# sourcedennis/wasm-pathtracer

Hardware: AMD Instinct MI355X
Metric: Mray/s (primary+shadow+bounce) at 1920x1080, 1/2/4/8 GPU; L2 vs CPU ref (higher is better)
Workload: dtype f32; 1 GPU; C3 bunny scene (scene id 2), 1920x1080, 64 spp per GPU share (64 spp frame), depth 8, NormalNEE; rays=25682600955, parallelism=single GPU

## Files before the change

include/wpt.h:

```cpp
#ifndef WPT_H
#define WPT_H

#include <stddef.h>
#include <stdint.h>

#ifdef __cplusplus
extern "C" {
#endif

#define WPT_OK 0
#define WPT_ERR_NOT_INIT (-1)
#define WPT_ERR_ALREADY_INIT (-2)
#define WPT_ERR_INVALID_SCENE (-3)
#define WPT_ERR_INVALID_ARG (-4)
#define WPT_ERR_UNSUPPORTED (-5)
#define WPT_ERR_DEVICE (-6)
#define WPT_ERR_NO_MESH (-7)

#define WPT_NO_NEE 0
#define WPT_NORMAL_NEE 1
#define WPT_PNEE 2


int wpt_init(uint32_t width, uint32_t height, uint32_t scene_id, float cam_x, float cam_y, float cam_z,
// ... 85 lines not shown
#define WPT_OPT_TRAVERSAL_SH 2
#define WPT_OPT_FUSED 3
#define WPT_OPT_FUSED_BELOW 4
#define WPT_OPT_SMALL_LANES 5
#define WPT_OPT_PIXEL_TILE 6
#define WPT_OPT_GRID_PCT 7
#define WPT_OPT_REFILL 8
#define WPT_OPT_REFILL_SH 9
#define WPT_OPT_TREELET 10
#define WPT_OPT_BVH_BUILD 11
#define WPT_OPT_LANES 12
#define WPT_OPT_FINISH_BELOW 13
#define WPT_OPT_TRACE_GRID_PCT 14
#define WPT_OPT_FINISH_EVERY 20
#define WPT_OPT_PROBE 22
#define WPT_OPT_STOCK 23
#define WPT_OPT_STOCK_LANES 24
#define WPT_OPT_FILL 25
#define WPT_OPT_ASYNC_PRIO 26
#define WPT_OPT_ASYNC_GRID_PCT 27
#define WPT_OPT_STOCK_AHEAD 30
#define WPT_OPT_STOCK_EVERY 32
#define WPT_OPT_STOCK_EXTRA 33
#define WPT_OPT_ASYNC_ONESHOT 31
#define WPT_OPT_STOCK_PREFILL 35
#define WPT_OPT_ASYNC_FUSED_BELOW 36
#define WPT_OPT_PRESOLVE 37
#define WPT_OPT_DROP_MISS 38
#define WPT_OPT_PRESOLVE_SHADOW 39
#define WPT_OPT_GEN_SHADE 40
#define WPT_OPT_STOCK_RANKS 42
#define WPT_OPT_STOCK_RING_BYTES 43
#define WPT_OPT_VIEWPORT 44
#define WPT_OPT_LOG 34
#define WPT_OPT_SCENE_TRAVERSAL 28
#define WPT_OPT_OCT_VIEW 41
#define WPT_OPT_SCENE_TRI_ONLY 29
int wpt_set_option(int32_t option, int64_t value);
int64_t wpt_probe_read(uint32_t* meta, uint32_t* rec, uint64_t* rec_entries, double* ticks_per_us);
int wpt_get_option(int32_t option, int64_t* value);
int wpt_scene_build_info(double* out);
int wpt_clear_stats(void);
int wpt_sync(void);
int wpt_bvh_depth(void);

int wpt_trace_rays(size_t n, const float* rays, float* t_out, int32_t* id_out);
int wpt_shadow_rays(size_t n, const float* pq, const int32_t* light, uint8_t* occluded);
int wpt_first_hit(uint32_t sample, float* dir3, float* t, int32_t* id, uint32_t* visits,
                  float* normal3, float* albedo3, uint8_t* kind);
int wpt_primary_rays(uint32_t width, uint32_t height, const float* cam5, uint32_t frame_seed,
                     uint32_t sample, float* rays6);
int wpt_presolve_rays(size_t n, const float* rays, uint8_t* resolved, float* t_out, int32_t* id_out);
int wpt_presolve_shadow_rays(size_t n, const float* pq, const int32_t* light, uint8_t* resolved);

int wpt_shutdown(void);

void* wpt_debug_scene_new(int32_t scene_id, const float* mesh_vertices, size_t num_vertices);
int wpt_debug_scene_info(void* h, uint64_t* out);
int wpt_debug_scene_nodes4(void* h, uint32_t* out);
int wpt_debug_scene_nodes(void* h, uint32_t* out);
int wpt_debug_scene_shapes(void* h, float* out);
int wpt_debug_scene_materials(void* h, float* out);
int wpt_debug_scene_lights(void* h, uint32_t* out);
int wpt_debug_scene_presolve(void* h, size_t n, const float* rays, uint8_t* resolved, float* t_out, int32_t* id_out);
int wpt_debug_scene_guards(void* h, uint32_t* num_guards, float* boxes, uint32_t* leaf_guard);
int wpt_debug_scene_presolve_shadow(void* h, size_t n, const float* pq, const int32_t* light, uint8_t* resolved);
// ... 11 lines not shown
```

wasm-pathtracer_amd/csrc/wpt_render.h:

```cpp
#pragma once
#include <hip/hip_runtime.h>
#include <stdint.h>
#include <string>
#include <algorithm>
#include <deque>
#include <vector>

#include "wpt_photon.h"
#include "wpt_scene.h"
#include "wpt_seqsum.h"

namespace wpt {

constexpr int kMaxInf = 16;
constexpr int kMaxBvhDepth = 4096;
constexpr int kMaxBounces = 512;

struct DevScene {
  const float4* nodes;
  const float4* tree;
  uint32_t tree_pairs, tree_root_lf;
  const float4* prims;
  const uint32_t* kinds;
  const float4* all;
  const uint32_t* all_kinds;
  const float4* mats;
  const float4* lights;
  const float4* nodes4;
  const uint32_t* leaf_table;
  uint32_t num_inf, num_finite, num_shapes, num_lights;
  uint32_t use_bvh, tri_only;
  uint32_t refill_lanes;
  uint32_t refill_lanes_sh;
  int stack_cap;
  uint32_t* overflow;
  const uint32_t* oct_child;
  const float* oct_cum;
  const uint32_t* oct_corners;
  uint32_t oct_nodes;
  uint32_t oct_lds_words;
  float bg[3];
  float4 planes[kMaxInf];
  uint4* probe;
  const PresolveBoxes* pre;
};

struct Stats {
  uint64_t paths = 0;
  uint64_t rays = 0;
  uint64_t shadow_rays = 0;
  uint64_t node_visits = 0;
  uint64_t prim_tests = 0;
  uint64_t bounces = 0;
  uint64_t ext_visits = 0, ext_tests = 0, ext_node_bytes = 0;
  uint64_t sh_visits = 0, sh_tests = 0, sh_node_bytes = 0;
  uint64_t fallback_ext = 0, fallback_sh = 0;
  uint64_t ex_body_lanes = 0, ex_bodies = 0, lf_body_lanes = 0, lf_bodies = 0;
  uint64_t ext_lane_iters = 0, ext_live_iters = 0, sh_lane_iters = 0, sh_live_iters = 0;
  uint64_t photon_rays = 0, photons = 0;
  uint64_t trace_bytes = 0;
  uint64_t max_ray_visits = 0;
  uint64_t sum_chunks = 0, sum_resummed = 0, sum_fetched = 0;
  uint64_t finish_paths = 0, finish_max_bounces = 0;
  uint64_t stock_traced = 0, stock_consumed = 0, fill_paths = 0;
  uint64_t stock_deficit = 0, stock_waits = 0, plan_us = 0, stock_us = 0;
  uint64_t stock_rays = 0;
  uint64_t stock_rays_used = 0;
// ... 349 lines not shown
  uint64_t xslot_ = 0;
  uint64_t maxpart_ = 0;
  uint32_t* d_xidx_ = nullptr;
  bool photons_ok_ = false;
  uint64_t photons_shot_ = 0, photons_stored_ = 0;
  std::vector<uint32_t> oct_child_;
  std::vector<float> oct_cum_;
  uint32_t* d_oct_child_ = nullptr;
  float* d_oct_cum_ = nullptr;
  uint32_t* d_oct_corners_ = nullptr;

  int device_ = -1;
  int ncu_ = 256;
  static constexpr int kTravVariants = 8;
  uint32_t grid_ext_[2 * kTravVariants] = {};
  uint32_t grid_sh_[2 * kTravVariants] = {};
  uint32_t grid_tr_[4] = {};
  uint32_t grid_shade_ = 512;
  uint32_t shade_occ_[32] = {};
  size_t shade_occ_smem_[32] = {};
  bool fused_ = false;
  uint64_t fused_below_ = 1ull << 24;
  int small_lanes_ = 2;
  int traversal_ = 3, traversal_sh_ = 3;
  int trav_ext_ = 0, trav_sh_ = 0;
  bool treelet_ = true;
  uint32_t pixel_tile_ = 8;
  int grid_pct_ = 50;
#ifndef WPT_TRACE_GRID_PCT
#define WPT_TRACE_GRID_PCT 75
#endif
  int trace_grid_pct_ = WPT_TRACE_GRID_PCT;
  uint32_t refill_ = 12, refill_sh_ = 16;
  uint64_t finish_below_ = 1u << 18;
  int finish_every_ = 4;
  uint32_t num_guards_ = 0;
  uint32_t light_guards_ = 0;
  bool presolve_ = true;
  bool drop_miss_ = true;
  bool presolve_shadow_ = true;
  bool gen_shade_ = true;
  uint32_t gen_shade_occ_[2] = {};
  uint32_t probe_cap_ = 0, probe_waves_ = 0, probe_used_ = 0;
  uint4* d_probe_ = nullptr;
  std::vector<uint32_t> probe_meta_;
  uint4* probe_slot(const LaunchCtx& C, int kernel, uint32_t grid);
  uint32_t* d_fallback_ = nullptr;
  void* d_fh_ = nullptr;
  size_t fh_cap_ = 0;
  uint2* d_fh_spill_ = nullptr;
  size_t fh_spill_cap_ = 0;
  hipStream_t stream_ = nullptr;
  PathSet lanes_[kMaxLanes];
  int lanes_made_ = 0;
  bool stats_pending_ = false;
  int pend_nl_ = 0, pend_b_ = 0;
  bool pend_stock_ = false, pend_presolve_ = false;
  int nlanes_ = 4;
  hipEvent_t ev_main_ = nullptr;
  hipEvent_t ev_ref_ = nullptr;
  std::vector<void*> scene_bufs_;
  DevScene ds_{};
  uint32_t depth_ = 0;
  bool scene_ok_ = false;

  uint32_t w_ = 0, h_ = 0;
// ... 38 lines not shown
```

wasm-pathtracer_amd/csrc/wpt_render.hip:

```cpp
#include "wpt_render.h"
#include "wpt_partition.h"
#include "wpt_photon.h"
#include "wpt_quartic.h"
#include "wpt_seqsum.h"

#include <algorithm>
#include <chrono>
#include <cstdlib>
#include <cmath>
#include <cstdio>
#include <cstring>
#include <deque>
#include <memory>
#include <mutex>
#include <unordered_map>
#include <thread>
#include <type_traits>

#define HIP_OK(expr)                                                     \
  do {                                                                   \
    hipError_t e_ = (expr);                                              \
    if (e_ != hipSuccess) {                                              \
      err = std::string(#expr " failed: ") + hipGetErrorString(e_);      \
      return false;                                                      \
// ... 301 lines not shown
  h.root_b = S.nodes[1];
  if (kTreePairs > 0) {
    for (uint32_t i = threadIdx.x; i < 4 * S.tree_pairs; i += kTBlock) {
      const float4 v = S.tree[i];
      tree[i] = f4v{v.x, v.y, v.z, v.w};
    }
    if (S.tree_pairs != 0) h.root_b.z = __uint_as_float(S.tree_root_lf);
  }
  h.gtree = gtree;
  const bool fits = S.num_lights <= kLdsLights;
  if (fits && threadIdx.x < 4 * S.num_lights) {
    const uint32_t l = threadIdx.x >> 2, w = threadIdx.x & 3u;
    const uint32_t sid = __float_as_uint(S.lights[5 * l + 1].w);
    const float4 v = S.prims[4 * (size_t)(sid - S.num_inf) + w];
    lrec[4 * threadIdx.x] = v.x;
    lrec[4 * threadIdx.x + 1] = v.y;
    lrec[4 * threadIdx.x + 2] = v.z;
    lrec[4 * threadIdx.x + 3] = v.w;
    if (w == 0) lid[l] = (int32_t)sid;
  }
  __syncthreads();
  h.lrec = fits ? lrec : nullptr;
  h.lid = lid;
  return h;
}

template <bool COUNT>
__device__ __forceinline__ bool enter_root(const DevScene& S, const Hot& H, Lane& L, uint32_t& visits,
                                           uint32_t& nbytes) {
  if (COUNT) { visits++; nbytes += 32; }
  const float4 a = H.root_a, b = H.root_b;
  float h;
  if (!box_entry(a, b, L.o, L.inv, L.best, h)) return false;
  L.lf = __float_as_uint(b.z);
  L.cnt = __float_as_uint(b.w);
  L.sp = 0;
  return true;
}

typedef __attribute__((address_space(3))) uint32_t lds_u32;
typedef __attribute__((address_space(3))) float lds_f32;
struct Stack {
  lds_u32* code;
  lds_f32* h;
  uint2* spill;
  uint32_t stride;
  int cap;
  uint32_t* overflow;
};

__device__ __forceinline__ uint32_t encode_child(uint32_t lf, uint32_t cnt, uint32_t node) {
  const uint32_t leaf = (cnt < 128u && lf < (1u << 24)) ? (0x80000000u | (cnt << 24) | lf) : (0x40000000u | node);
  return cnt == 0 ? lf : leaf;
}

__device__ __forceinline__ void stack_store(const Stack& st, int k, uint32_t code, float h) {
  if (k < kLdsSlots) {
    st.code[k * kTBlock] = code;
    st.h[k * kTBlock] = h;
  } else {
    st.spill[(size_t)(k - kLdsSlots) * st.stride] = make_uint2(code, __float_as_uint(h));
  }
}

__device__ __forceinline__ void stack_load(const Stack& st, int k, uint32_t& code, float& h) {
  if (k < kLdsSlots) {
    code = st.code[k * kTBlock];
    h = st.h[k * kTBlock];
// ... 1058 lines not shown
    cnt[0] = (uint32_t)__popcll(fm);
    const OutMasks M = count_out<true>(R, V, cnt + 1);
    cnt[4] = ShadeFields::pack((uint32_t)__popcll(__ballot(drop0)), (uint32_t)__popcll(__ballot(shaded)));
    if (lane == 0) A.publish(wid, cnt);
    __syncthreads();
    if (wid == 0)
      A.reserve(lane,
                {{3, false, ~0u}, {0, false, ~0u}, {0, true, ~0u}, {1, false, ShadeFields::kMask}, {-1, false, 0u}},
                [&](const uint32_t(&incl)[5]) {
                  const uint32_t tf = A.total(incl[0]), te = A.total(incl[4]);
                  auto t = shade_take<BA>(lane, reinterpret_cast<u64*>(counts + 2), incl[1], incl[2], A.total(incl[3]));
                  if (lane == kWaves + 2)
                    t = A.take(counts, tf, 0u, true);
                  else if (lane == kWaves + 3)
                    t = A.take(counts + kResWord, 0u, ShadeFields::get(te, 0), true);
                  else if (lane == kWaves + 4)
                    t = A.take(counts + kGenShadeWord, ShadeFields::top(te, 1), 0u, true);
                  t.go = t.go && t.inc != 0ull;
                  return t;
                });
    __syncthreads();
    if (front0) {
      const uint32_t p = A.at(0, wid, (uint32_t)__popcll(fm & below));
      s0.thr[p] = R.th;
      s0.o[p] = R.ro;
      s0.d[p] = R.rd;
    } else
      store_out<true, 1>(A, wid, below, M, R, V, out, sh, col, t_nx, id_nx, n);
    __syncthreads();
  }
}

struct WaveFeed {
  uint32_t n, v, wave, nwaves;
  __device__ WaveFeed(uint32_t n_) : n(n_), v(0) {
    wave = (blockIdx.x * kTBlock + threadIdx.x) >> 6;
    nwaves = (gridDim.x * kTBlock) >> 6;
  }
  static constexpr uint32_t K = kFeedChunk;
  __device__ uint32_t pos(uint32_t k) const { return ((k / K) * nwaves + wave) * K + (k % K); }
  __device__ bool more() const { return pos(v) < n; }
  __device__ uint32_t taken() const { return taken_below(n); }
  __device__ uint32_t taken_below(uint32_t m) const {
    const uint32_t C = m / K, rem = m % K;
    const uint32_t full = C > wave ? (C - wave - 1u) / nwaves + 1u : 0u;
    const uint32_t part = (rem != 0u && C % nwaves == wave) ? rem : 0u;
    return min(v, full * K + part);
  }
  __device__ uint32_t take(uint64_t take_m) {
    const uint32_t rank = (uint32_t)__popcll(take_m & ((1ull << (threadIdx.x & 63)) - 1ull));
    const uint32_t p = pos(v + rank);
    v += (uint32_t)__popcll(take_m);
    return p;
  }
};

template <int OCT>
__global__ void __launch_bounds__(kShadeBlock) k_photon_sample(DevScene S, uint32_t n, const float* __restrict__ pts,
                                                               const uint32_t* __restrict__ st_in,
                                                               uint32_t* __restrict__ light, float* __restrict__ pdf,
                                                               uint32_t* __restrict__ st_out) {
  extern __shared__ uint32_t s_oct[];
  const OctView<OCT> O = oct_view<OCT>(S, s_oct);
  __syncthreads();
  for (uint32_t i = blockIdx.x * kShadeBlock + threadIdx.x; i < n; i += gridDim.x * kShadeBlock) {
    uint32_t s = st_in[i], li = 0;
    float p = 0.0f;
    photon_sample(S, O, s, mk(pts[3 * (size_t)i], pts[3 * (size_t)i + 1], pts[3 * (size_t)i + 2]), li, p);
    light[i] = li;
    pdf[i] = p;
    st_out[i] = s;
  }
}

__global__ void __launch_bounds__(kBlock) k_photon_gen(DevScene S, uint32_t seed, uint32_t k0, uint32_t n,
                                                       float4* __restrict__ ro, float4* __restrict__ rd,
                                                       float4* __restrict__ rec) {
  const uint32_t i = blockIdx.x * kBlock + threadIdx.x;
  if (i >= n) return;
  uint32_t s = photon_seed(seed, k0 + i);
  const uint32_t li = xs_next_in_range(s, S.num_lights);
  const float4* L = S.lights + 5 * (size_t)li;
  const float4 L0 = L[0], L1 = L[1], L2 = L[2], L3 = L[3], L4 = L[4];
  const float q1 = xs_next(s);
  const float q2 = xs_next(s);
  const float q1s = sqrtf(q1);
// ... 65 lines not shown
    const uint32_t f = (uint32_t)__popcll(__ballot(live && L.cnt != 0));
    ex_lanes += e;
    ex_bodies += e ? 1u : 0u;
    lf_lanes += f;
    lf_bodies += f ? 1u : 0u;
  }
  __device__ __forceinline__ void flush(unsigned long long* work, int ca, int cb) const {
    work_add_wave(work, ca, 64ull * it);
    work_add_wave(work, ca + 1, live_a);
    if (cb >= 0) {
      work_add_wave(work, cb, 64ull * it);
      work_add_wave(work, cb + 1, live_b);
    }
    work_add_wave(work, 10, ex_lanes);
    work_add_wave(work, 11, ex_bodies);
    work_add_wave(work, 12, lf_lanes);
    work_add_wave(work, 13, lf_bodies);
  }
};

template <bool TRI_ONLY, bool COUNT, int TRAV>
__global__ void WPT_TRACE_BOUNDS k_extend(DevScene S, const float4* __restrict__ ro,
                                                   const float4* __restrict__ rd, const uint32_t* __restrict__ count,
                                                   float* __restrict__ t_out, int32_t* __restrict__ id_out,
                                                   uint2* __restrict__ spill, unsigned long long* work,
                                                   uint32_t* fallbacks) {
  constexpr bool FAST = TRAV == 1;
  __shared__ uint32_t s_code[kLdsSlots * kTBlock];
  __shared__ float s_h[kLdsSlots * kTBlock];
  __shared__ float s_lrec[16 * kLdsLights];
  __shared__ int32_t s_lid[kLdsLights];
  __shared__ f4v s_tree[4 * kTreePairs + 1];
  const uint32_t n = *count;
  const Hot H = load_hot(S, (lds_f32h*)s_lrec, (lds_i32*)s_lid, (lds_f4v*)s_tree, (const float4*)s_tree);
  const uint32_t G = gridDim.x * kTBlock;
  const Stack stk{(lds_u32*)(s_code + threadIdx.x), (lds_f32*)(s_h + threadIdx.x),
                  spill + blockIdx.x * kTBlock + threadIdx.x, G, S.stack_cap, S.overflow};
  uint32_t visits = 0, tests = 0, nbytes = 0;
  WaveFeed feed(n);
  const uint32_t p_t0 = S.probe ? probe_now() : 0u;
  uint32_t p_dry = 0u;
  Lane L;
  uint32_t slot = 0;
  bool live = false;
  bool fast = FAST;
  bool tie = false, quirk = false, dummy = false;
  BodyLanes bodies;
  const float inf = __int_as_float(0x7f800000);
  for (;;) {
    const uint64_t idle_m = __ballot(!live);
    const uint32_t nidle = (uint32_t)__popcll(idle_m);
    if (nidle != 0 && (nidle >= S.refill_lanes || nidle == 64u) && feed.more()) {
      const uint32_t q0 = feed.take(idle_m);
      const bool got = q0 < n;
      if (S.probe && p_dry == 0u && !feed.more()) p_dry = probe_now();
      if (!live && got) {
        slot = q0;
        fast = FAST;
        tie = quirk = false;
        const float4 o4 = ro[slot], d4 = rd[slot];
        live = begin_extend<TRI_ONLY, COUNT, FAST>(S, H, L, ld3(o4), ld3(d4), visits, tests, nbytes);
        if (!live) st_hit(t_out + slot, id_out + slot, L.best_id >= 0 ? L.best : inf, L.best_id);
      }
    }
    if (!__any(live) && !feed.more()) {
      if (S.probe) probe_close(S, p_t0, p_dry, feed.taken());
      break;
    }
    if (COUNT) bodies.count(live, false, L);
    if (live) {
      const bool more = (FAST && fast)
                            ? step4<false, TRI_ONLY, COUNT>(S, L, stk, -1, 0.0f, dummy, tie, quirk, visits, tests, nbytes)
                            : step<false, TRI_ONLY, COUNT>(S, H, L, stk, -1, 0.0f, dummy, visits, tests, nbytes);
      if (!more) {
        live = false;
        if (FAST && fast && (tie || quirk)) {
          fast = false;
          atomicAdd(fallbacks, 1u);
          live = begin_extend<TRI_ONLY, COUNT, false>(S, H, L, L.o, L.d, visits, tests, nbytes);
        }
        if (!live) st_hit(t_out + slot, id_out + slot, L.best_id >= 0 ? L.best : inf, L.best_id);
      }
    }
  }
  if (COUNT) {
    work_add(work, 0, visits);
    work_add(work, 1, tests);
    work_add(work, 2, nbytes);
    bodies.flush(work, 6, -1);
  }
}

__device__ __forceinline__ void add_contribution(float4* __restrict__ col, float4 c) {
  const uint32_t path = __float_as_uint(c.w);
  float4 v = col[path];
  v.x += c.x;
  v.y += c.y;
  v.z += c.z;
  col[path] = v;
}

template <bool TRI_ONLY, bool COUNT, int TRAV>
__global__ void WPT_TRACE_BOUNDS k_shadow(DevScene S, const uint32_t* __restrict__ count,
                                                   const float4* __restrict__ so, const float4* __restrict__ sd,
                                                   const float4* __restrict__ sc, float4* __restrict__ col,
                                                   uint8_t* __restrict__ occ_out, uint2* __restrict__ spill,
                                                   unsigned long long* work, uint32_t* fallbacks) {
  constexpr bool FAST = TRAV == 1;
  __shared__ uint32_t s_code[kLdsSlots * kTBlock];
  __shared__ float s_h[kLdsSlots * kTBlock];
  __shared__ float s_lrec[16 * kLdsLights];
  __shared__ int32_t s_lid[kLdsLights];
  __shared__ f4v s_tree[4 * kTreePairs + 1];
  const uint32_t n = *count;
  const Hot H = load_hot(S, (lds_f32h*)s_lrec, (lds_i32*)s_lid, (lds_f4v*)s_tree, (const float4*)s_tree);
  const uint32_t G = gridDim.x * kTBlock;
  const Stack stk{(lds_u32*)(s_code + threadIdx.x), (lds_f32*)(s_h + threadIdx.x),
                  spill + blockIdx.x * kTBlock + threadIdx.x, G, S.stack_cap, S.overflow};
  uint32_t visits = 0, tests = 0, nbytes = 0;
  WaveFeed feed(n);
  const uint32_t p_t0 = S.probe ? probe_now() : 0u;
  uint32_t p_dry = 0u;
  Lane L;
  uint32_t cur = 0;
  float dir_len = 0.0f, early = 0.0f;
  int32_t light = -1;
  bool occluded = false;
  bool live = false;
  bool fast = FAST;
  bool tie = false, quirk = false;
  BodyLanes bodies;
  for (;;) {
    bool finished = false;
    const uint64_t idle_m = __ballot(!live);
    const uint32_t nidle = (uint32_t)__popcll(idle_m);
    if (nidle != 0 && (nidle >= S.refill_lanes_sh || nidle == 64u) && feed.more()) {
      const uint32_t q0 = feed.take(idle_m);
      const bool got = q0 < n;
      if (S.probe && p_dry == 0u && !feed.more()) p_dry = probe_now();
      if (!live && got) {
        cur = q0;
        const float4 o4 = so[cur], d4 = sd[cur];
        dir_len = o4.w;
        light = (int32_t)__float_as_uint(d4.w);
        fast = FAST;
        tie = quirk = false;
        live = begin_shadow<TRI_ONLY, COUNT, FAST>(S, H, L, ld3(o4), ld3(d4), dir_len, light, early, occluded, visits,
                                                   tests, nbytes);
        finished = !live;
      }
    }
    if (!__any(live || finished) && !feed.more()) {
      if (S.probe) probe_close(S, p_t0, p_dry, feed.taken());
      break;
    }
    if (COUNT) bodies.count(live, false, L);
    if (live) {
      const bool more =
          (FAST && fast)
              ? step4<true, TRI_ONLY, COUNT>(S, L, stk, light, early, occluded, tie, quirk, visits, tests, nbytes)
              : step<true, TRI_ONLY, COUNT>(S, H, L, stk, light, early, occluded, visits, tests, nbytes);
      if (!more) {
        live = false;
        finished = true;
        if (FAST && fast && !occluded && (tie || quirk)) {
          fast = false;
          atomicAdd(fallbacks + 1, 1u);
          if (begin_shadow<TRI_ONLY, COUNT, false>(S, H, L, L.o, L.d, dir_len, light, early, occluded, visits, tests,
                                                   nbytes)) {
            live = true;
            finished = false;
          }
// ... 2 lines not shown
    }
    if (finished) {
      const bool occ = shadow_verdict(L, dir_len, light, occluded);
      if (occ_out) occ_out[cur] = occ ? 1 : 0;
      else if (!occ) add_contribution(col, sc[cur]);
    }
  }
  if (COUNT) {
    work_add(work, 3, visits);
    work_add(work, 4, tests);
    work_add(work, 5, nbytes);
    bodies.flush(work, 8, -1);
  }
}

template <bool TRI_ONLY, bool COUNT>
#ifndef WPT_FUSED_WAVES
#define WPT_FUSED_WAVES 8
#endif
__global__ void __launch_bounds__(kTBlock, TRI_ONLY ? WPT_FUSED_WAVES : 1) k_trace(DevScene S, const float4* __restrict__ ro,
                                                  const float4* __restrict__ rd, const uint32_t* __restrict__ cnt_ext,
                                                  float* __restrict__ t_out, int32_t* __restrict__ id_out,
                                                  const uint32_t* __restrict__ cnt_sh, const float4* __restrict__ so,
                                                  const float4* __restrict__ sd, const float4* __restrict__ sc,
                                                  float4* __restrict__ col, uint2* __restrict__ spill,
                                                  unsigned long long* work) {
  __shared__ uint32_t s_code[kLdsSlots * kTBlock];
  __shared__ float s_h[kLdsSlots * kTBlock];
  __shared__ float s_lrec[16 * kLdsLights];
  __shared__ int32_t s_lid[kLdsLights];
  __shared__ f4v s_tree[4 * kTreePairs + 1];
  const uint32_t ne = *cnt_ext;
  const uint32_t n = ne + *cnt_sh;
  const Hot H = load_hot(S, (lds_f32h*)s_lrec, (lds_i32*)s_lid, (lds_f4v*)s_tree, (const float4*)s_tree);
  const uint32_t G = gridDim.x * kTBlock;
  const Stack stk{(lds_u32*)(s_code + threadIdx.x), (lds_f32*)(s_h + threadIdx.x),
                  spill + blockIdx.x * kTBlock + threadIdx.x, G, S.stack_cap, S.overflow};
  uint32_t ev = 0, et = 0, eb = 0, sv = 0, st = 0, sb = 0, cv = 0, ct = 0, cb = 0, vmax = 0;
  WaveFeed feed(n);
  const uint32_t p_t0 = S.probe ? probe_now() : 0u;
  uint32_t p_dry = 0u;
  Lane L;
  uint32_t slot = 0;
  bool live = false, is_sh = false, occluded = false;
  BodyLanes bodies;
  float dir_len = 0.0f, early = -__int_as_float(0x7f800000);
  int32_t light = -1;
  const float inf = __int_as_float(0x7f800000);
  for (;;) {
    bool finished = false;
    const uint64_t idle_m = __ballot(!live);
    const uint32_t nidle = (uint32_t)__popcll(idle_m);
    if (nidle != 0 && (nidle >= S.refill_lanes || nidle == 64u) && feed.more()) {
      const uint32_t q0 = feed.take(idle_m);
      const bool got = q0 < n;
      if (!live && got) {
        is_sh = q0 >= ne;
        slot = is_sh ? q0 - ne : q0;
      }
      if (S.probe && p_dry == 0u && !feed.more()) p_dry = probe_now();
      if (!live && got) {
        const float4 o4 = is_sh ? so[slot] : ro[slot];
        const float4 d4 = is_sh ? sd[slot] : rd[slot];
        if (!is_sh) {
          light = -1;
          early = -inf;
          occluded = false;
          live = begin_extend<TRI_ONLY, COUNT, false>(S, H, L, ld3(o4), ld3(d4), cv, ct, cb);
        } else {
          dir_len = o4.w;
          light = (int32_t)__float_as_uint(d4.w);
          live = begin_shadow<TRI_ONLY, COUNT, false>(S, H, L, ld3(o4), ld3(d4), dir_len, light, early, occluded, cv,
                                                      ct, cb);
        }
        finished = !live;
      }
    }
    if (!__any(live || finished) && !feed.more()) {
      if (S.probe) probe_close(S, p_t0, p_dry, feed.taken());
      break;
    }
    if (COUNT) bodies.count(live, is_sh, L);
    if (live) {
      if (!step<true, TRI_ONLY, COUNT>(S, H, L, stk, light, early, occluded, cv, ct, cb)) {
        live = false;
        finished = true;
      }
    }
    if (finished) {
      if (!is_sh) st_hit(t_out + slot, id_out + slot, L.best_id >= 0 ? L.best : inf, L.best_id);
      else if (!shadow_verdict(L, dir_len, light, occluded)) add_contribution(col, sc[slot]);
      if (COUNT) {
        vmax = max(vmax, cv);
// ... 470 lines not shown
  if (!up(all.data(), all.size() * sizeof(float4), &p)) return false;
  ds.all = (const float4*)p;
  if (!up(all_kinds.data(), all_kinds.size() * sizeof(uint32_t), &p)) return false;
  ds.all_kinds = (const uint32_t*)p;
  if (!up(mats.data(), mats.size() * sizeof(float4), &p)) return false;
  ds.mats = (const float4*)p;
  if (!up(lights.data(), lights.size() * sizeof(float4), &p)) return false;
  ds.lights = (const float4*)p;
  {
    const size_t n4 = std::max<size_t>(sc.nodes4.size(), 1);
    std::vector<Node4> n4v(n4);
    if (!sc.nodes4.empty()) memcpy(n4v.data(), sc.nodes4.data(), sizeof(Node4) * sc.nodes4.size());
    if (!up(n4v.data(), sizeof(Node4) * n4, &p)) return false;
    ds.nodes4 = (const float4*)p;
    std::vector<uint32_t> lt(std::max<size_t>(sc.leaf_table.size(), 2), 0u);
    std::copy(sc.leaf_table.begin(), sc.leaf_table.end(), lt.begin());
    if (!up(lt.data(), sizeof(uint32_t) * lt.size(), &p)) return false;
    ds.leaf_table = (const uint32_t*)p;
    auto mode = [&](int want) {
      const bool b4 = want == 1 || (want == 3 && !sc.tri_only && sc.use_bvh);
      return (b4 && !sc.nodes4.empty()) ? 1 : 0;
    };
    trav_ext_ = mode(traversal_);
    trav_sh_ = mode(traversal_sh_);
  }
  ds.num_inf = sc.num_inf;
  ds.num_finite = (uint32_t)nf;
  ds.num_shapes = (uint32_t)ns;
  ds.num_lights = (uint32_t)sc.lights.size();
  ds.use_bvh = sc.use_bvh ? 1u : 0u;
  ds.tri_only = sc.tri_only ? 1u : 0u;
  ds.refill_lanes = refill_;
  ds.refill_lanes_sh = refill_sh_;
  for (int k = 0; k < 3; k++) ds.bg[k] = sc.background[k];
  for (uint32_t i = 0; i < sc.num_inf && i < (uint32_t)kMaxInf; i++) ds.planes[i] = all[4 * i];
  {
    PresolveBoxes pre{};
    if (sc.use_bvh && nf != 0) pre = sc.pre;
    if (!up(&pre, sizeof pre, &p)) return false;
    ds.pre = (const PresolveBoxes*)p;
    num_guards_ = pre.num_guards;
    light_guards_ = pre.light_guards;
  }
  ds_ = ds;
  depth_ = sc.depth;
  ds_.stack_cap = (int)std::max<uint32_t>(sc.depth + 2, 3 * sc.depth4 + 4);
  ds_.overflow = d_fallback_ + 2;
  if (!size_grids(err)) return false;
  scene_ok_ = true;
  return true;
}

bool Renderer::set_option(int opt, int64_t v, std::string& err) {
  auto range = [&](int64_t lo, int64_t hi) {
    if (v < lo || v > hi) {
      err = "option value out of range";
      return false;
    }
    return true;
  };
  switch (opt) {
    case 1:
    case 2:
      if (!range(0, 3) || v == 2) { err = "traversal: 0 (bvh2), 1 (bvh4) or 3 (auto)"; return false; }
      (opt == 1 ? traversal_ : traversal_sh_) = (int)v;
      return true;
// ... 11 lines not shown
    case 12:
      if (!set_lanes((int)v)) { err = "lanes out of range"; return false; }
      return true;
    case 13: if (!range(0, (int64_t)1 << 32)) return false; finish_below_ = (uint64_t)v; return true;
    case 14:
      if (!range(1, 100)) return false;
      trace_grid_pct_ = (int)v;
      return !stream_ || size_grids(err);
    case 20: if (!range(1, 64)) return false; finish_every_ = (int)v; return true;
    case 23:
      if (v != 0 && (v < 64 || v > 4096 || (v & (v - 1)) != 0)) { err = "stock: 0 or a power of two 64..4096"; return false; }
      if (!drain_async(err)) return false;
      stock_drop();
      stock_slots_ = (uint32_t)v;
      return true;
    case 42:
      if (!range(0, 1)) return false;
      if (!drain_async(err)) return false;
      stock_drop();
      stock_ranks_ = v != 0;
      return true;
    case 25: if (!range(0, 1)) return false; fill_on_ = v != 0; return true;
    case 30: if (!range(0, 64)) return false; stock_ahead_ = (uint32_t)v; return true;
    case 32: if (!range(1, 1024)) return false; stock_every_ = (uint32_t)v; return true;
    case 33: if (!range(0, 64)) return false; stock_extra_ = (uint32_t)v; return true;
    case 31: if (!range(0, 1)) return false; async_oneshot_ = v != 0; return true;
    case 34: if (!range(0, 1)) return false; log_ = (int)v; return true;
    case 35: if (!range(0, 1)) return false; stock_prefill_ = v != 0; return true;
    case 36: if (!range(0, (int64_t)1 << 40)) return false; async_fused_below_ = (uint64_t)v; return true;
    case 37: if (!range(0, 1)) return false; presolve_ = v != 0; return true;
    case 38: if (!range(0, 1)) return false; drop_miss_ = v != 0; return true;
    case 39: if (!range(0, 1)) return false; presolve_shadow_ = v != 0; return true;
    case 40: if (!range(0, 1)) return false; gen_shade_ = v != 0; return true;
    case 26:
      if (!range(0, 1)) return false;
      if (!drain_async(err)) return false;
      async_prio_ = (int)v;
      return true;
    case 27: if (!range(0, 100)) return false; async_grid_pct_ = (int)v; return true;
    case 28:
    case 29:
    case 41:
    case 43:
    case 44: err = "read-only option"; return false;
    case 24:
      if (!range(1, kMaxLanes - kAsyncLane0 - 1)) return false;
      if (!drain_async(err)) return false;
      stock_lanes_ = (int)v;
      refill_lane_ = 0;
      return true;
    case 22:
      if (!range(0, 1 << 20)) return false;
      probe_cap_ = (uint32_t)v;
      probe_used_ = 0;
      probe_meta_.clear();
      if (d_probe_) { (void)hipFree(d_probe_); d_probe_ = nullptr; }
      return true;
    default: err = "unknown option"; return false;
  }
}

bool Renderer::get_option(int opt, int64_t& v) const {
  switch (opt) {
    case 1: v = traversal_; return true;
    case 2: v = traversal_sh_; return true;
    case 3: v = fused_ ? 1 : 0; return true;
    case 4: v = (int64_t)fused_below_; return true;
    case 5: v = small_lanes_; return true;
    case 6: v = pixel_tile_; return true;
    case 7: v = grid_pct_; return true;
    case 8: v = refill_; return true;
    case 9: v = refill_sh_; return true;
    case 10: v = treelet_ ? 1 : 0; return true;
    case 12: v = nlanes_; return true;
    case 13: v = (int64_t)finish_below_; return true;
    case 14: v = trace_grid_pct_; return true;
    case 20: v = finish_every_; return true;
    case 22: v = probe_cap_; return true;
    case 23: v = stock_slots_; return true;
    case 25: v = fill_on_ ? 1 : 0; return true;
    case 30: v = stock_ahead_; return true;
    case 32: v = stock_every_; return true;
    case 33: v = stock_extra_; return true;
    case 31: v = async_oneshot_ ? 1 : 0; return true;
    case 34: v = log_; return true;
    case 35: v = stock_prefill_ ? 1 : 0; return true;
    case 36: v = (int64_t)async_fused_below_; return true;
    case 37: v = presolve_ ? 1 : 0; return true;
    case 38: v = drop_miss_ ? 1 : 0; return true;
    case 39: v = presolve_shadow_ ? 1 : 0; return true;
    case 40: v = gen_shade_ ? 1 : 0; return true;
    case 26: v = async_prio_; return true;
    case 27: v = async_grid_pct_; return true;
    case 28: v = !scene_ok_ ? -1 : !ds_.use_bvh ? 2 : trav_ext_; return true;
    case 29: v = !scene_ok_ ? -1 : ds_.tri_only ? 1 : 0; return true;
    case 41: v = !photons_ok_ ? -1 : ds_.oct_lds_words == 0 ? 0 : (ds_.oct_lds_words > ds_.oct_nodes ? 2 : 1); return true;
    case 24: v = stock_lanes_; return true;
    case 42: v = stock_ranks_ ? 1 : 0; return true;
    case 43: v = (int64_t)ring_bytes(); return true;
    case 44: v = (int64_t)w_ | ((int64_t)h_ << 32); return true;
    default: return false;
  }
}

bool Renderer::set_viewport(uint32_t w, uint32_t h, std::string& err) {
  if (!stream_) { err = "no device"; return false; }
  if (w == 0 || h == 0) { err = "empty viewport"; return false; }
  if (!drain_async(err)) return false;
  stock_drop();
  HIP_OK(hipStreamSynchronize(stream_));
  w_ = w;
  h_ = h;
  free_rounds();
  if (d_acc_) (void)hipFree(d_acc_);
  if (d_cnt_) (void)hipFree(d_cnt_);
  if (d_rgba_) (void)hipFree(d_rgba_);
  if (d_samp_) (void)hipFree(d_samp_);
  d_acc_ = nullptr; d_cnt_ = nullptr; d_rgba_ = nullptr; d_samp_ = nullptr;
  HIP_OK(hipMalloc(&d_acc_, sizeof(float4) * (size_t)w * h));
  HIP_OK(hipMalloc(&d_cnt_, sizeof(uint32_t) * (size_t)w * h));
  HIP_OK(hipMalloc(&d_rgba_, 4 * (size_t)w * h));
  HIP_OK(hipMalloc(&d_samp_, 4 * (size_t)w * h));
  return set_partition(rank_, nranks_, tile_, err);
}
// ... 1188 lines not shown
}

bool Renderer::read_radiance(float* acc3, uint32_t* cnt, std::string& err) {
  const size_t np = (size_t)w_ * h_;
  std::vector<float4> a(np);
  HIP_OK(hipMemcpyAsync(a.data(), d_acc_, sizeof(float4) * np, hipMemcpyDeviceToHost, stream_));
  if (cnt) HIP_OK(hipMemcpyAsync(cnt, d_cnt_, sizeof(uint32_t) * np, hipMemcpyDeviceToHost, stream_));
  HIP_OK(hipStreamSynchronize(stream_));
  for (size_t i = 0; i < np; i++) {
    acc3[3 * i] = a[i].x;
    acc3[3 * i + 1] = a[i].y;
    acc3[3 * i + 2] = a[i].z;
  }
  return true;
}

bool Renderer::copy_partition(float* dev_dst, std::string& err) {
  const uint32_t n = (uint32_t)part_pix_.size();
  k_pack_partition<<<blocks_for(n), kBlock, 0, stream_>>>(nranks_ > 1 ? d_part_pix_ : nullptr, n, d_acc_, d_cnt_,
                                                          (float4*)dev_dst);
  HIP_OK(hipGetLastError());
  HIP_OK(hipStreamSynchronize(stream_));
  return true;
}

bool Renderer::launch_extend(const LaunchCtx& C, const float4* ro, const float4* rd, const uint32_t* cnt,
                             std::string& err) {
  const PathSet& L = *C.ps;
  const int v = (ds_.tri_only ? 1 : 0) | (C.count ? 2 : 0) | (trav_ext_ << 2);
  const int full = C.batch_lanes == 1 ? kTravVariants : 0;
  const uint32_t g = std::min(async_grid(C, grid_ext_[v + full], 100), spill_grid(L));
  DevScene ds = ds_;
  ds.probe = probe_slot(C, 1, g);
#define WPT_EXT(T, CN, F)                                                                                     \
  k_extend<T, CN, F><<<g, kTBlock, 0, C.stream>>>(ds, ro, rd, cnt, L.hit_t(C.hit_sel), L.hit_id(C.hit_sel), \
                                                 L.spill, d_work_, d_fallback_)
  switch (v) {
    case 0: LAUNCH_TIMED(C, 1, extend, n_extend, WPT_EXT(false, false, 0)); break;
    case 1: LAUNCH_TIMED(C, 1, extend, n_extend, WPT_EXT(true, false, 0)); break;
    case 2: LAUNCH_TIMED(C, 1, extend, n_extend, WPT_EXT(false, true, 0)); break;
    case 3: LAUNCH_TIMED(C, 1, extend, n_extend, WPT_EXT(true, true, 0)); break;
    case 4: LAUNCH_TIMED(C, 1, extend, n_extend, WPT_EXT(false, false, 1)); break;
    case 5: LAUNCH_TIMED(C, 1, extend, n_extend, WPT_EXT(true, false, 1)); break;
    case 6: LAUNCH_TIMED(C, 1, extend, n_extend, WPT_EXT(false, true, 1)); break;
    default: LAUNCH_TIMED(C, 1, extend, n_extend, WPT_EXT(true, true, 1)); break;
  }
#undef WPT_EXT
  if (ds.probe && C.probe_res) {
    k_probe_add<<<1, 1, 0, C.stream>>>(ds.probe, C.probe_res);
    if (C.bounce == 0) k_probe_add_sh<<<1, 1, 0, C.stream>>>(ds.probe, L.counts + kGenShadeWord);
    HIP_OK(hipGetLastError());
  }
  return true;
}

bool Renderer::launch_shadow(const LaunchCtx& C, const uint32_t* cnt, uint8_t* occ_out, std::string& err) {
  const PathSet& L = *C.ps;
  const int v = (ds_.tri_only ? 1 : 0) | (C.count ? 2 : 0) | (trav_sh_ << 2);
  const int full = C.batch_lanes == 1 ? kTravVariants : 0;
  const uint32_t g = std::min(async_grid(C, grid_sh_[v + full], 100), spill_grid(L));
  DevScene ds = ds_;
  ds.probe = probe_slot(C, 3, g);
#define WPT_SH(T, CN, F)                                                                                        \
  k_shadow<T, CN, F><<<g, kTBlock, 0, C.stream>>>(ds, cnt, L.so, L.sd, L.sc, L.col, occ_out, L.spill, d_work_, \
                                                 d_fallback_)
  switch (v) {
    case 0: LAUNCH_TIMED(C, 3, shadow, n_shadow, WPT_SH(false, false, 0)); break;
    case 1: LAUNCH_TIMED(C, 3, shadow, n_shadow, WPT_SH(true, false, 0)); break;
    case 2: LAUNCH_TIMED(C, 3, shadow, n_shadow, WPT_SH(false, true, 0)); break;
    case 3: LAUNCH_TIMED(C, 3, shadow, n_shadow, WPT_SH(true, true, 0)); break;
    case 4: LAUNCH_TIMED(C, 3, shadow, n_shadow, WPT_SH(false, false, 1)); break;
    case 5: LAUNCH_TIMED(C, 3, shadow, n_shadow, WPT_SH(true, false, 1)); break;
    case 6: LAUNCH_TIMED(C, 3, shadow, n_shadow, WPT_SH(false, true, 1)); break;
    default: LAUNCH_TIMED(C, 3, shadow, n_shadow, WPT_SH(true, true, 1)); break;
  }
#undef WPT_SH
  if (ds.probe && C.probe_res) {
    k_probe_add_sh<<<1, 1, 0, C.stream>>>(ds.probe, cnt + (kShResWord - 3));
    HIP_OK(hipGetLastError());
  }
  return true;
}

bool Renderer::launch_trace(const LaunchCtx& C, std::string& err) {
  const PathSet& L = *C.ps;
  const int b = C.bounce;
  const int v = (ds_.tri_only ? 1 : 0) | (C.count ? 2 : 0);
  const uint32_t g = std::min(async_grid(C, grid_tr_[v], trace_grid_pct_, 2), spill_grid(L));
  DevScene ds = ds_;
  ds.probe = probe_slot(C, 5, g);
#define WPT_TR(T, CN)                                                                                          \
  k_trace<T, CN><<<g, kTBlock, 0, C.stream>>>(ds, L.ro[b & 1], L.rd[b & 1], L.ext_count(b), L.hit_t(C.hit_sel), \
                                             L.hit_id(C.hit_sel), L.sh_count(b - 1), L.so, L.sd, L.sc, L.col,  \
                                             L.spill, d_work_)
  switch (v) {
    case 0: LAUNCH_TIMED(C, 5, trace, n_trace, WPT_TR(false, false)); break;
    case 1: LAUNCH_TIMED(C, 5, trace, n_trace, WPT_TR(true, false)); break;
    case 2: LAUNCH_TIMED(C, 5, trace, n_trace, WPT_TR(false, true)); break;
    default: LAUNCH_TIMED(C, 5, trace, n_trace, WPT_TR(true, true)); break;
  }
#undef WPT_TR
  if (ds.probe && C.probe_res) {
    k_probe_add<<<1, 1, 0, C.stream>>>(ds.probe, C.probe_res);
    k_probe_add_sh<<<1, 1, 0, C.stream>>>(ds.probe, L.sh_count(b - 1) + (kShResWord - 3));
    HIP_OK(hipGetLastError());
  }
  return true;
}

uint4* Renderer::probe_slot(const LaunchCtx& C, int kernel, uint32_t grid) {
  if (probe_used_ >= probe_cap_) return nullptr;
  const uint32_t waves = grid * (kTBlock / 64);
  if (!d_probe_) {
    probe_waves_ = max_grid() * (kTBlock / 64);
    const uint64_t cap_max = (1ull << 28) / std::max<uint32_t>(probe_waves_, 1);
    probe_cap_ = (uint32_t)std::min<uint64_t>(probe_cap_, cap_max);
    if (hipMalloc(&d_probe_, sizeof(uint4) * (size_t)probe_waves_ * probe_cap_) != hipSuccess) {
      d_probe_ = nullptr;
      probe_cap_ = 0;
      return nullptr;
    }
  }
  if (waves > probe_waves_) return nullptr;
// ... 827 lines not shown
```

wasm-pathtracer_amd/interface.py:

```python
import ctypes

import numpy as np

from ._lib import lib

OK = 0
ERR_NOT_INIT, ERR_ALREADY_INIT, ERR_INVALID_SCENE, ERR_INVALID_ARG = -1, -2, -3, -4
ERR_UNSUPPORTED, ERR_DEVICE, ERR_NO_MESH = -5, -6, -7
NO_NEE, NORMAL_NEE, PNEE = 0, 1, 2


class WptError(RuntimeError):
    def __init__(self, code, msg):
        super().__init__(f"[{code}] {msg}")
        self.code = code


def _check(rc):
    if rc < 0:
        raise WptError(rc, lib().wpt_last_error().decode())
    return rc


def init(width, height, scene_id, cam_x, cam_y, cam_z, cam_rot_x, cam_rot_y):
# ... 241 lines not shown
    out = (ctypes.c_double * 28)()
    _check(lib().wpt_kernel_times(ctypes.addressof(out), 28))
    names = ("generate", "extend", "shade", "shadow", "accumulate", "trace")
    kt = {n: {"ms": out[2 * i], "launches": int(out[2 * i + 1]), "busy_ms": out[12 + 2 * i],
              "logical_launches": int(out[13 + 2 * i])} for i, n in enumerate(names)}
    return kt


def set_counting(on):
    _check(lib().wpt_set_counting(1 if on else 0))


def set_profiling(on):
    _check(lib().wpt_set_profiling(1 if on else 0))


def scene_build_info():
    out = (ctypes.c_double * 2)()
    _check(lib().wpt_scene_build_info(ctypes.addressof(out)))
    return float(out[0]), bool(out[1])


def set_lanes(n):
    _check(lib().wpt_set_lanes(int(n)))


OPTIONS = {"defaults": 0, "traversal": 1, "traversal_sh": 2, "fused": 3, "fused_below": 4, "small_lanes": 5, "pixel_tile": 6,
           "grid_pct": 7, "refill": 8, "refill_sh": 9, "treelet": 10, "bvh_build": 11, "lanes": 12,
           "finish_below": 13, "trace_grid_pct": 14, "finish_every": 20, "probe": 22, "stock": 23, "stock_lanes": 24,
           "fill": 25, "async_prio": 26, "async_grid_pct": 27, "scene_traversal": 28, "scene_tri_only": 29,
           "stock_ahead": 30, "async_oneshot": 31, "stock_every": 32, "stock_extra": 33,
           "log": 34, "stock_prefill": 35, "async_fused_below": 36, "presolve": 37, "drop_miss": 38,
           "presolve_shadow": 39, "gen_shade": 40, "oct_view": 41,
           "stock_ranks": 42, "stock_ring_bytes": 43, "viewport": 44}
TRAVERSALS = {"bvh2": 0, "bvh4": 1, "auto": 3}
OPTION_VALUES = {"traversal": TRAVERSALS, "traversal_sh": TRAVERSALS,
                 "bvh_build": {"auto": 0, "host": 1, "gpu": 2}}


def set_option(name, value):
    if isinstance(value, str) and not value.lstrip("-").isdigit():
        value = OPTION_VALUES[name][value]
    _check(lib().wpt_set_option(OPTIONS[name], int(value)))


def get_option(name):
    v = ctypes.c_int64(0)
    _check(lib().wpt_get_option(OPTIONS[name], ctypes.addressof(v)))
    return v.value


def probe_read():
    L = lib()
    ent = ctypes.c_uint64(0)
    tpu = ctypes.c_double(0.0)
    n = L.wpt_probe_read(None, None, ctypes.addressof(ent), ctypes.addressof(tpu))
    if n < 0:
        raise WptError(int(n), L.wpt_last_error().decode())
    meta = np.zeros((n, 5), np.uint32)
    rec = np.zeros((ent.value, 4), np.uint32)
    if n:
        ent.value = rec.shape[0]
        _check(L.wpt_probe_read(meta.ctypes.data, rec.ctypes.data, ctypes.addressof(ent), ctypes.addressof(tpu)))
    return meta, rec, tpu.value


def clear_stats():
# ... 157 lines not shown
```

Before: 10090 Mray/s.

## Size wave feed to work count and retire surplus blocks early

```diff
diff --git a/include/wpt.h b/include/wpt.h
--- a/include/wpt.h
+++ b/include/wpt.h
@@ -141,6 +141,7 @@
 #define WPT_OPT_STOCK_RANKS 42
 #define WPT_OPT_STOCK_RING_BYTES 43
 #define WPT_OPT_VIEWPORT 44
+#define WPT_OPT_FEED_MIN_CHUNKS 45
 #define WPT_OPT_LOG 34
 #define WPT_OPT_SCENE_TRAVERSAL 28
 #define WPT_OPT_OCT_VIEW 41
diff --git a/wasm-pathtracer_amd/csrc/wpt_feed.h b/wasm-pathtracer_amd/csrc/wpt_feed.h
--- /dev/null
+++ b/wasm-pathtracer_amd/csrc/wpt_feed.h
@@ -0,0 +1,39 @@
+#pragma once
+#include <stdint.h>
+
+#if defined(__HIPCC__)
+#include <hip/hip_runtime.h>
+#define WPT_FEED_HD __host__ __device__ __forceinline__
+#else
+#define WPT_FEED_HD inline
+#endif
+
+namespace wpt {
+
+constexpr uint32_t kFeedMinChunksMax = 4096;
+
+WPT_FEED_HD uint32_t feed_waves(uint32_t n, uint32_t nwaves, uint32_t block_waves, uint32_t c, uint32_t K) {
+  const uint32_t per = K * c;
+  const uint32_t want = n / per + (n % per != 0u ? 1u : 0u);
+  const uint32_t blocks = want > block_waves ? (want + block_waves - 1u) / block_waves : 1u;
+  const uint32_t wa = blocks * block_waves;
+  return wa < nwaves ? wa : nwaves;
+}
+
+WPT_FEED_HD uint32_t feed_pos(uint32_t wa, uint32_t w, uint32_t k, uint32_t K) {
+  return ((k / K) * wa + w) * K + (k % K);
+}
+
+WPT_FEED_HD uint32_t feed_taken_below(uint32_t wa, uint32_t w, uint32_t v, uint32_t m, uint32_t K) {
+  const uint32_t C = m / K, rem = m % K;
+  const uint32_t full = C > w ? (C - w - 1u) / wa + 1u : 0u;
+  const uint32_t part = (rem != 0u && C % wa == w) ? rem : 0u;
+  const uint32_t own = full * K + part;
+  return v < own ? v : own;
+}
+
+WPT_FEED_HD uint32_t feed_own(uint32_t wa, uint32_t w, uint32_t n, uint32_t K) {
+  return feed_taken_below(wa, w, 0xFFFFFFFFu, n, K);
+}
+
+}
diff --git a/wasm-pathtracer_amd/csrc/wpt_render.h b/wasm-pathtracer_amd/csrc/wpt_render.h
--- a/wasm-pathtracer_amd/csrc/wpt_render.h
+++ b/wasm-pathtracer_amd/csrc/wpt_render.h
@@ -6,6 +6,7 @@
 #include <deque>
 #include <vector>
 
+#include "wpt_feed.h"
 #include "wpt_photon.h"
 #include "wpt_scene.h"
 #include "wpt_seqsum.h"
@@ -33,6 +34,7 @@
   uint32_t refill_lanes;
   uint32_t refill_lanes_sh;
   int stack_cap;
+  uint32_t feed_min_chunks;
   uint32_t* overflow;
   const uint32_t* oct_child;
   const float* oct_cum;
@@ -448,6 +450,8 @@
 #endif
   int trace_grid_pct_ = WPT_TRACE_GRID_PCT;
   uint32_t refill_ = 12, refill_sh_ = 16;
+  uint32_t feed_min_chunks_ = 1;
+  uint32_t feed_chunks(const LaunchCtx& C) const { return C.async && async_oneshot_ ? 1u : feed_min_chunks_; }
   uint64_t finish_below_ = 1u << 18;
   int finish_every_ = 4;
   uint32_t num_guards_ = 0;
diff --git a/wasm-pathtracer_amd/csrc/wpt_render.hip b/wasm-pathtracer_amd/csrc/wpt_render.hip
--- a/wasm-pathtracer_amd/csrc/wpt_render.hip
+++ b/wasm-pathtracer_amd/csrc/wpt_render.hip
@@ -357,8 +357,14 @@
   const float4 a = H.root_a, b = H.root_b;
   float h;
   if (!box_entry(a, b, L.o, L.inv, L.best, h)) return false;
-  L.lf = __float_as_uint(b.z);
-  L.cnt = __float_as_uint(b.w);
+  if (S.tree_pairs != 0) {
+    L.lf = S.tree_root_lf;
+    L.cnt = 0;
+  } else {
+    const float4 rb = S.nodes[1];
+    L.lf = __float_as_uint(rb.z);
+    L.cnt = __float_as_uint(rb.w);
+  }
   L.sp = 0;
   return true;
 }
@@ -1483,26 +1489,25 @@
 }
 
 struct WaveFeed {
-  uint32_t n, v, wave, nwaves;
-  __device__ WaveFeed(uint32_t n_) : n(n_), v(0) {
-    wave = (blockIdx.x * kTBlock + threadIdx.x) >> 6;
-    nwaves = (gridDim.x * kTBlock) >> 6;
+  uint32_t own, v, base, row;
+  __device__ WaveFeed(uint32_t n, uint32_t min_chunks) : v(0) {
+    const uint32_t wave = (uint32_t)__builtin_amdgcn_readfirstlane((int)((blockIdx.x * kTBlock + threadIdx.x) >> 6));
+    const uint32_t wa = feed_waves(n, (gridDim.x * kTBlock) >> 6, kTBlock >> 6, min_chunks, K);
+    own = wave < wa ? feed_own(wa, wave, n, K) : 0u;
+    base = wave * K;
+    row = wa * 64u;
   }
   static constexpr uint32_t K = kFeedChunk;
-  __device__ uint32_t pos(uint32_t k) const { return ((k / K) * nwaves + wave) * K + (k % K); }
-  __device__ bool more() const { return pos(v) < n; }
-  __device__ uint32_t taken() const { return taken_below(n); }
-  __device__ uint32_t taken_below(uint32_t m) const {
-    const uint32_t C = m / K, rem = m % K;
-    const uint32_t full = C > wave ? (C - wave - 1u) / nwaves + 1u : 0u;
-    const uint32_t part = (rem != 0u && C % nwaves == wave) ? rem : 0u;
-    return min(v, full * K + part);
-  }
+  static constexpr uint32_t kNone = 0xFFFFFFFFu;
+  __device__ bool idle_block() const { return blockIdx.x * kTBlock >= row; }
+  __device__ uint32_t lanes() const { return row; }
+  __device__ bool more() const { return v < own; }
+  __device__ uint32_t taken() const { return min(v, own); }
+  __device__ uint32_t taken_below(uint32_t m) const { return feed_taken_below(row / 64u, base / K, v, m, K); }
   __device__ uint32_t take(uint64_t take_m) {
-    const uint32_t rank = (uint32_t)__popcll(take_m & ((1ull << (threadIdx.x & 63)) - 1ull));
-    const uint32_t p = pos(v + rank);
+    const uint32_t k = v + (uint32_t)__popcll(take_m & ((1ull << (threadIdx.x & 63)) - 1ull));
     v += (uint32_t)__popcll(take_m);
-    return p;
+    return k < own ? (k / K) * (row / 64u * K) + base + (k % K) : kNone;
   }
 };
 
@@ -1634,14 +1639,18 @@
   __shared__ int32_t s_lid[kLdsLights];
   __shared__ f4v s_tree[4 * kTreePairs + 1];
   const uint32_t n = *count;
+  WaveFeed feed(n, S.feed_min_chunks);
+  const uint32_t p_t0 = S.probe ? probe_now() : 0u;
+  if (feed.idle_block()) {
+    if (S.probe) probe_close(S, p_t0, 0u, 0u);
+    return;
+  }
+  uint32_t p_dry = 0u;
   const Hot H = load_hot(S, (lds_f32h*)s_lrec, (lds_i32*)s_lid, (lds_f4v*)s_tree, (const float4*)s_tree);
-  const uint32_t G = gridDim.x * kTBlock;
+  const uint32_t G = feed.lanes();
   const Stack stk{(lds_u32*)(s_code + threadIdx.x), (lds_f32*)(s_h + threadIdx.x),
                   spill + blockIdx.x * kTBlock + threadIdx.x, G, S.stack_cap, S.overflow};
   uint32_t visits = 0, tests = 0, nbytes = 0;
-  WaveFeed feed(n);
-  const uint32_t p_t0 = S.probe ? probe_now() : 0u;
-  uint32_t p_dry = 0u;
   Lane L;
   uint32_t slot = 0;
   bool live = false;
@@ -1654,8 +1663,8 @@
     const uint32_t nidle = (uint32_t)__popcll(idle_m);
     if (nidle != 0 && (nidle >= S.refill_lanes || nidle == 64u) && feed.more()) {
       const uint32_t q0 = feed.take(idle_m);
-      const bool got = q0 < n;
-      if (S.probe && p_dry == 0u && !feed.more()) p_dry = probe_now();
+      const bool got = q0 != WaveFeed::kNone;
+      if (S.probe && !feed.more()) p_dry = probe_now();
       if (!live && got) {
         slot = q0;
         fast = FAST;
@@ -1715,14 +1724,18 @@
   __shared__ int32_t s_lid[kLdsLights];
   __shared__ f4v s_tree[4 * kTreePairs + 1];
   const uint32_t n = *count;
+  WaveFeed feed(n, S.feed_min_chunks);
+  const uint32_t p_t0 = S.probe ? probe_now() : 0u;
+  if (feed.idle_block()) {
+    if (S.probe) probe_close(S, p_t0, 0u, 0u);
+    return;
+  }
+  uint32_t p_dry = 0u;
   const Hot H = load_hot(S, (lds_f32h*)s_lrec, (lds_i32*)s_lid, (lds_f4v*)s_tree, (const float4*)s_tree);
-  const uint32_t G = gridDim.x * kTBlock;
+  const uint32_t G = feed.lanes();
   const Stack stk{(lds_u32*)(s_code + threadIdx.x), (lds_f32*)(s_h + threadIdx.x),
                   spill + blockIdx.x * kTBlock + threadIdx.x, G, S.stack_cap, S.overflow};
   uint32_t visits = 0, tests = 0, nbytes = 0;
-  WaveFeed feed(n);
-  const uint32_t p_t0 = S.probe ? probe_now() : 0u;
-  uint32_t p_dry = 0u;
   Lane L;
   uint32_t cur = 0;
   float dir_len = 0.0f, early = 0.0f;
@@ -1738,8 +1751,8 @@
     const uint32_t nidle = (uint32_t)__popcll(idle_m);
     if (nidle != 0 && (nidle >= S.refill_lanes_sh || nidle == 64u) && feed.more()) {
       const uint32_t q0 = feed.take(idle_m);
-      const bool got = q0 < n;
-      if (S.probe && p_dry == 0u && !feed.more()) p_dry = probe_now();
+      const bool got = q0 != WaveFeed::kNone;
+      if (S.probe && !feed.more()) p_dry = probe_now();
       if (!live && got) {
         cur = q0;
         const float4 o4 = so[cur], d4 = sd[cur];
@@ -1808,14 +1821,18 @@
   __shared__ f4v s_tree[4 * kTreePairs + 1];
   const uint32_t ne = *cnt_ext;
   const uint32_t n = ne + *cnt_sh;
+  WaveFeed feed(n, S.feed_min_chunks);
+  const uint32_t p_t0 = S.probe ? probe_now() : 0u;
+  if (feed.idle_block()) {
+    if (S.probe) probe_close(S, p_t0, 0u, 0u);
+    return;
+  }
+  uint32_t p_dry = 0u;
   const Hot H = load_hot(S, (lds_f32h*)s_lrec, (lds_i32*)s_lid, (lds_f4v*)s_tree, (const float4*)s_tree);
-  const uint32_t G = gridDim.x * kTBlock;
+  const uint32_t G = feed.lanes();
   const Stack stk{(lds_u32*)(s_code + threadIdx.x), (lds_f32*)(s_h + threadIdx.x),
                   spill + blockIdx.x * kTBlock + threadIdx.x, G, S.stack_cap, S.overflow};
   uint32_t ev = 0, et = 0, eb = 0, sv = 0, st = 0, sb = 0, cv = 0, ct = 0, cb = 0, vmax = 0;
-  WaveFeed feed(n);
-  const uint32_t p_t0 = S.probe ? probe_now() : 0u;
-  uint32_t p_dry = 0u;
   Lane L;
   uint32_t slot = 0;
   bool live = false, is_sh = false, occluded = false;
@@ -1829,12 +1846,12 @@
     const uint32_t nidle = (uint32_t)__popcll(idle_m);
     if (nidle != 0 && (nidle >= S.refill_lanes || nidle == 64u) && feed.more()) {
       const uint32_t q0 = feed.take(idle_m);
-      const bool got = q0 < n;
+      const bool got = q0 != WaveFeed::kNone;
       if (!live && got) {
         is_sh = q0 >= ne;
         slot = is_sh ? q0 - ne : q0;
       }
-      if (S.probe && p_dry == 0u && !feed.more()) p_dry = probe_now();
+      if (S.probe && !feed.more()) p_dry = probe_now();
       if (!live && got) {
         const float4 o4 = is_sh ? so[slot] : ro[slot];
         const float4 d4 = is_sh ? sd[slot] : rd[slot];
@@ -2371,6 +2388,7 @@
   ds.tri_only = sc.tri_only ? 1u : 0u;
   ds.refill_lanes = refill_;
   ds.refill_lanes_sh = refill_sh_;
+  ds.feed_min_chunks = feed_min_chunks_;
   for (int k = 0; k < 3; k++) ds.bg[k] = sc.background[k];
   for (uint32_t i = 0; i < sc.num_inf && i < (uint32_t)kMaxInf; i++) ds.planes[i] = all[4 * i];
   {
@@ -2448,6 +2466,11 @@
     case 38: if (!range(0, 1)) return false; drop_miss_ = v != 0; return true;
     case 39: if (!range(0, 1)) return false; presolve_shadow_ = v != 0; return true;
     case 40: if (!range(0, 1)) return false; gen_shade_ = v != 0; return true;
+    case 45:
+      if (!range(1, kFeedMinChunksMax)) return false;
+      feed_min_chunks_ = (uint32_t)v;
+      ds_.feed_min_chunks = feed_min_chunks_;
+      return true;
     case 26:
       if (!range(0, 1)) return false;
       if (!drain_async(err)) return false;
@@ -2506,6 +2529,7 @@
     case 38: v = drop_miss_ ? 1 : 0; return true;
     case 39: v = presolve_shadow_ ? 1 : 0; return true;
     case 40: v = gen_shade_ ? 1 : 0; return true;
+    case 45: v = feed_min_chunks_; return true;
     case 26: v = async_prio_; return true;
     case 27: v = async_grid_pct_; return true;
     case 28: v = !scene_ok_ ? -1 : !ds_.use_bvh ? 2 : trav_ext_; return true;
@@ -3760,6 +3784,7 @@
   const uint32_t g = std::min(async_grid(C, grid_ext_[v + full], 100), spill_grid(L));
   DevScene ds = ds_;
   ds.probe = probe_slot(C, 1, g);
+  ds.feed_min_chunks = feed_chunks(C);
 #define WPT_EXT(T, CN, F)                                                                                     \
   k_extend<T, CN, F><<<g, kTBlock, 0, C.stream>>>(ds, ro, rd, cnt, L.hit_t(C.hit_sel), L.hit_id(C.hit_sel), \
                                                  L.spill, d_work_, d_fallback_)
@@ -3789,6 +3814,7 @@
   const uint32_t g = std::min(async_grid(C, grid_sh_[v + full], 100), spill_grid(L));
   DevScene ds = ds_;
   ds.probe = probe_slot(C, 3, g);
+  ds.feed_min_chunks = feed_chunks(C);
 #define WPT_SH(T, CN, F)                                                                                        \
   k_shadow<T, CN, F><<<g, kTBlock, 0, C.stream>>>(ds, cnt, L.so, L.sd, L.sc, L.col, occ_out, L.spill, d_work_, \
                                                  d_fallback_)
@@ -3817,6 +3843,7 @@
   const uint32_t g = std::min(async_grid(C, grid_tr_[v], trace_grid_pct_, 2), spill_grid(L));
   DevScene ds = ds_;
   ds.probe = probe_slot(C, 5, g);
+  ds.feed_min_chunks = feed_chunks(C);
 #define WPT_TR(T, CN)                                                                                          \
   k_trace<T, CN><<<g, kTBlock, 0, C.stream>>>(ds, L.ro[b & 1], L.rd[b & 1], L.ext_count(b), L.hit_t(C.hit_sel), \
                                              L.hit_id(C.hit_sel), L.sh_count(b - 1), L.so, L.sd, L.sc, L.col,  \
diff --git a/wasm-pathtracer_amd/interface.py b/wasm-pathtracer_amd/interface.py
--- a/wasm-pathtracer_amd/interface.py
+++ b/wasm-pathtracer_amd/interface.py
@@ -297,7 +297,8 @@
            "stock_ahead": 30, "async_oneshot": 31, "stock_every": 32, "stock_extra": 33,
            "log": 34, "stock_prefill": 35, "async_fused_below": 36, "presolve": 37, "drop_miss": 38,
            "presolve_shadow": 39, "gen_shade": 40, "oct_view": 41,
-           "stock_ranks": 42, "stock_ring_bytes": 43, "viewport": 44}
+           "stock_ranks": 42, "stock_ring_bytes": 43, "viewport": 44,
+           "feed_min_chunks": 45}
 TRAVERSALS = {"bvh2": 0, "bvh4": 1, "auto": 3}
 OPTION_VALUES = {"traversal": TRAVERSALS, "traversal_sh": TRAVERSALS,
                  "bvh_build": {"auto": 0, "host": 1, "gpu": 2}}
```

New measurement: 10110 Mray/s (median of 3 runs). No clear change (+0.1%).
